# ShuoYangRobotics/Cerberus

Measured on NVIDIA H100. Metric: sliding-window solves/sec (10-frame x 150-feature windows), higher is better.
Workload: dtype f64

## Files before the change

cerberus_b200/csrc/solve_kernel.cuh:

```cuda
#pragma once
#include "eval_kernels.cuh"

namespace cerb {

#if defined(CERB_PHASE_TIMING) && !defined(CERB_CUSIM)
__device__ unsigned long long g_phase_cycles[48];
#define PH_DECL() long long ph_t = clock64()
#define PH_MARK_T(id, t) do { if ((threadIdx.x & 31) == 0) { const long long ph_n = clock64(); if (threadIdx.x == (t)) atomicAdd(&g_phase_cycles[id], (unsigned long long)(ph_n - ph_t)); ph_t = ph_n; } __syncwarp(); } while (0)
#define PH_MARK(id) PH_MARK_T(id, 0)
#define PH_ARG , long long &ph_t
#define PH_FWD , ph_t
#else
#define PH_DECL()
#define PH_MARK_T(id, t)
#define PH_MARK(id)
#define PH_ARG
#define PH_FWD
#endif

enum { CERB_WINDOW = 10, NX = 79, NYB = 13, NFR = 11, NY = 143, NR = 222, NRP = 224, HXX_SZ = 79 * 79, HXY_SZ = 79 * 143, X_TD = 78, SOLVE_THREADS = 256, FT = 64, TILE_LD = 33, NOBS_PLANES = 9 };
enum { HBLK = NYB * NYB, AD_SZ = NFR * HBLK, BO_SZ = (NFR - 1) * HBLK };
#ifndef CERB_SOLVE_MIN_BLOCKS
#define CERB_SOLVE_MIN_BLOCKS 1
#endif
// ... 629 lines not shown
                    _Pragma("unroll")
                    for (int t = 0; t < 15; t++) {
                        const int o = plx[hq + t] + i * (ply[hq + t] & 4095);
                        const double nv = cur[t] + acc[(hq + t) >> 1][(hq + t) & 1];
                        smem_base[o] = nv;
                        smem_base[o + (ply[hq + t] >> 12) - 256] = nv;
                    }
                }
                PH_MARK(35);
            } else if (i + 1 < CERB_WINDOW && rnd < 3) load_S(i + 1);
            CERB_BAR_SYNC(2, 32 * IMU_WARPS);
            PH_MARK(36);
        }
        PH_MARK(30);
    } else {
        const int *meta = P.prior_meta + (size_t)w * PRIOR_META_STRIDE;
        if (meta[0]) {
            const int t5 = tid - 32 * IMU_WARPS, n = meta[1], nb = meta[2];
            const double *J = P.prior_J + (size_t)w * PRIOR_LD * PRIOR_LD, *r0 = P.prior_r + (size_t)w * PRIOR_LD, *x0 = P.prior_x0 + (size_t)w * 16 * 9;
            if (t5 < nb) {
                const int kind = meta[4 + 3 * t5], index = meta[5 + 3 * t5], col = meta[6 + 3 * t5];
                prior_block_dx(kind, x + prior_block_state_offset(kind, index), x0 + 9 * t5, s.pdx + col);
            }
            CERB_BAR_SYNC(3, PRIOR_THREADS);
            const int kc = (n + 1) / 2;
            for (int e = t5; e < 2 * n; e += PRIOR_THREADS) {
                const int p = e / n, i = e % n;
                const int k1 = (p + 1) * kc < n ? (p + 1) * kc : n;
                double t = 0.0;
                for (int k = p * kc; k < k1; k++) t += J[(size_t)k * n + i] * s.pdx[k];
                ppart[p * PRIOR_LD + i] = t;
            }
            CERB_BAR_SYNC(3, PRIOR_THREADS);
            for (int i = t5; i < n; i += PRIOR_THREADS) {
                const double t = (r0[i] + ppart[i]) + ppart[PRIOR_LD + i];
                s.pr[i] = t; cost += 0.5 * t * t;
            }
            CERB_BAR_SYNC(3, PRIOR_THREADS);
            for (int c = wid - IMU_WARPS; c < n; c += PRIOR_THREADS / 32) {
                double t = 0.0;
                for (int k = lane; k < n; k += 32) t += J[(size_t)c * n + k] * s.pr[k];
                for (int o = 16; o > 0; o >>= 1) t += __shfl_sync(0xffffffffu, t, (lane + o) & 31);
                const int d = s.ti[TI_PRIOR_MAP + c];
                if (lane == 0) gp[d >= 0 ? d : NX + (-d - 1)] += t;
            }
        }
        PH_MARK_T(31, 96);
    }
    __syncthreads();
    PH_MARK(26);
    for (int k = tid; k < NR; k += SOLVE_THREADS) s.g[k] += gp[k];
    __syncthreads();
    PH_MARK(27);
    return cost;
}

CERB_D void apply_plus(const Smem &s, const double *delta, const double *lam, const double *dlam, double *lamc, int nF, bool ex_open, bool td_open, int tid) {
    if (tid < 11) pose_plus(s.xs + ST_POSE + 7 * tid, delta + 6 * tid, s.xc + ST_POSE + 7 * tid);
    else if (tid < 13) {
        const int e = tid - 11;
        if (ex_open) pose_plus(s.xs + ST_EX + 7 * e, delta + 66 + 6 * e, s.xc + ST_EX + 7 * e);
        else for (int k = 0; k < 7; k++) s.xc[ST_EX + 7 * e + k] = s.xs[ST_EX + 7 * e + k];
    }
    for (int k = tid; k < 99; k += SOLVE_THREADS) { const int f = k / 9, c = k % 9; s.xc[ST_SB + k] = s.xs[ST_SB + k] + delta[NX + NYB * f + c]; }
    for (int k = tid; k < 44; k += SOLVE_THREADS) { const int f = k / 4, c = k % 4; s.xc[ST_LB + k] = s.xs[ST_LB + k] + delta[NX + NYB * f + 9 + c]; }
    if (tid == 0) s.xc[ST_TD] = td_open ? s.xs[ST_TD] + delta[X_TD] : s.xs[ST_TD];
    for (int f = tid; f < nF; f += SOLVE_THREADS) lamc[f] = lam[f] + dlam[f];
    __syncthreads();
}

CERB_D double ambient_sq(const double *a, const double *b, const double *la, const double *lb, int nF, bool ex_open, bool lb_open, bool td_open, int tid) {
    double t = 0.0;
    for (int k = tid; k < ST_SIZE; k += SOLVE_THREADS) {
        if (k >= ST_LB && k < ST_EX && !lb_open) continue;
        if (k >= ST_EX && k < ST_TD && !ex_open) continue;
        if (k == ST_TD && !td_open) continue;
        const double v = b ? a[k] - b[k] : a[k];
        t += v * v;
    }
    for (int f = tid; f < nF; f += SOLVE_THREADS) { const double v = lb ? la[f] - lb[f] : la[f]; t += v * v; }
    return t;
}

template <int W> struct TTPlan;
#define CERB_TT_PLAN(W, NR_, NB_, ...) template <> struct TTPlan<W> { static constexpr int nr = NR_, nb = NB_; static CERB_HD int tab(int i) { constexpr int t[] = {__VA_ARGS__}; return t[i]; } };
CERB_TT_PLAN(0, 4, 7, 0, 1, 2, 3, 0, 0, 0,   0, 0, 1, 0, 1, 0, 1,   0, 1, 1, 2, 2, 3, 3)
CERB_TT_PLAN(1, 4, 7, 2, 3, 4, 5, 0, 0, 0,   0, 0, 1, 0, 1, 0, 1,   0, 1, 1, 2, 2, 3, 3)
CERB_TT_PLAN(2, 4, 7, 4, 5, 6, 7, 0, 0, 0,   0, 0, 1, 0, 1, 0, 1,   0, 1, 1, 2, 2, 3, 3)
CERB_TT_PLAN(3, 4, 7, 6, 7, 8, 9, 0, 0, 0,   0, 0, 1, 0, 1, 0, 1,   0, 1, 1, 2, 2, 3, 3)
CERB_TT_PLAN(4, 6, 7, 8, 9, 0, 1, 4, 5, 0,   0, 0, 1, 2, 3, 2, 3,   0, 1, 1, 4, 4, 5, 5)
CERB_TT_PLAN(5, 6, 7, 0, 1, 6, 7, 8, 9, 0,   0, 0, 0, 0, 1, 1, 1,   2, 3, 4, 5, 2, 3, 4)
CERB_TT_PLAN(6, 7, 7, 1, 9, 2, 6, 7, 8, 3,   0, 2, 2, 2, 2, 6, 6,   1, 3, 4, 5, 1, 3, 4)
CERB_TT_PLAN(7, 5, 6, 3, 4, 5, 8, 9, 0, 0,   0, 0, 1, 1, 2, 2, 0,   3, 4, 3, 4, 3, 4, 0)
template <int W> CERB_D void ttt_warp(Smem &s, int lane) {
    typedef TTPlan<W> PL;
    const double *pr[7];
    _Pragma("unroll")
    for (int u = 0; u < 7; u++) {
        const int r = 8 * PL::tab(u < PL::nr ? u : 0) + (lane >> 2);
        pr[u] = (r < NX ? s.Hxy + r * NY : s.yv + NX) + (lane & 3);
    }
    double acc[7][2], fv[7];
    _Pragma("unroll")
    for (int k = 0; k < 7; k++) { acc[k][0] = 0.0; acc[k][1] = 0.0; }
    _Pragma("unroll")
    for (int u = 0; u < 7; u++) fv[u] = (u < PL::nr) ? pr[u][0] : 0.0;
    for (int q0 = 0; q0 < NY; q0 += 4) {
        const int qn = q0 + 4;
        const bool take = qn < NY && qn + (lane & 3) < NY;
        double fn[7];
        _Pragma("unroll")
        for (int u = 0; u < 7; u++) fn[u] = (u < PL::nr && take) ? pr[u][qn] : 0.0;
        _Pragma("unroll")
        for (int k = 0; k < 7; k++) if (k < PL::nb) CERB_DMMA(acc[k][0], acc[k][1], fv[PL::tab(7 + k)], fv[PL::tab(14 + k)], acc[k][0], acc[k][1]);
        _Pragma("unroll")
        for (int u = 0; u < 7; u++) fv[u] = fn[u];
    }
    _Pragma("unroll")
    for (int k = 0; k < 7; k++) {
        if (k >= PL::nb) continue;
        const int ba = PL::tab(PL::tab(7 + k)), bb = PL::tab(PL::tab(14 + k));
        const int a = 8 * ba + (lane >> 2);
        for (int e = 0; e < 2; e++) {
            const int b = 8 * bb + 2 * (lane & 3) + e;
            if (a > b || a >= NX || b > NX) continue;
            if (b == NX) s.yv[a] -= acc[k][e];
            else s.Hxx[b * NX + a] -= acc[k][e];
        }
    }
}

template <int W> struct SCPlan;
#define CERB_SC_PLAN(W, NR_, NB_, ...) template <> struct SCPlan<W> { static constexpr int nr = NR_, nb = NB_; static CERB_HD int tab(int i) { constexpr int t[] = {__VA_ARGS__}; return t[i]; } };
CERB_SC_PLAN(0, 8, 8, 0, 1, 2, 3, 4, 5, 6, 7, 0,   0, 0, 0, 0, 0, 0, 0, 0,   0, 1, 2, 3, 4, 5, 6, 7)
CERB_SC_PLAN(1, 9, 8, 0, 8, 9, 1, 2, 3, 4, 5, 6,   0, 0, 3, 3, 3, 3, 3, 3,   1, 2, 3, 4, 5, 6, 7, 8)
CERB_SC_PLAN(2, 9, 8, 1, 7, 8, 9, 2, 3, 4, 5, 6,   0, 0, 0, 4, 4, 4, 4, 4,   1, 2, 3, 4, 5, 6, 7, 8)
CERB_SC_PLAN(3, 8, 8, 2, 7, 8, 9, 3, 4, 5, 6, 0,   0, 0, 0, 4, 4, 4, 4, 4,   1, 2, 3, 4, 5, 6, 7, 1)
CERB_SC_PLAN(4, 7, 8, 3, 8, 9, 4, 5, 6, 7, 0, 0,   0, 0, 3, 3, 3, 3, 3, 3,   1, 2, 3, 4, 5, 6, 1, 2)
CERB_SC_PLAN(5, 5, 8, 5, 6, 7, 8, 9, 0, 0, 0, 0,   0, 0, 0, 0, 0, 1, 1, 1,   0, 1, 2, 3, 4, 1, 2, 3)
CERB_SC_PLAN(6, 4, 7, 6, 7, 8, 9, 0, 0, 0, 0, 0,   0, 1, 1, 1, 2, 2, 3, 0,   3, 1, 2, 3, 2, 3, 3, 0)
enum { SC_LDW = 36 };
template <int W> CERB_D void schur_tile(const double *tw, double (&acc)[8][2], int lane) {
    typedef SCPlan<W> PL;
    const double *pr[9];
    _Pragma("unroll")
    for (int u = 0; u < 9; u++) pr[u] = tw + (8 * PL::tab(u < PL::nr ? u : 0) + (lane >> 2)) * SC_LDW + (lane & 3);
    double fv[9];
    _Pragma("unroll")
    for (int u = 0; u < 9; u++) fv[u] = (u < PL::nr) ? pr[u][0] : 0.0;
    _Pragma("unroll")
    for (int ks = 0; ks < 8; ks++) {
        double fn[9];
        _Pragma("unroll")
        for (int u = 0; u < 9; u++) fn[u] = (u < PL::nr && ks < 7) ? pr[u][4 * (ks + 1)] : 0.0;
        _Pragma("unroll")
        for (int k = 0; k < 8; k++) if (k < PL::nb) CERB_DMMA(acc[k][0], acc[k][1], fv[PL::tab(9 + k)], fv[PL::tab(17 + k)], acc[k][0], acc[k][1]);
        _Pragma("unroll")
        for (int u = 0; u < 9; u++) fv[u] = fn[u];
    }
}
template <int W> CERB_D void schur_scatter(Smem &s, const double (&acc)[8][2], int lane) {
    typedef SCPlan<W> PL;
    _Pragma("unroll")
    for (int k = 0; k < 8; k++) {
        if (k >= PL::nb) continue;
        const int a = 8 * PL::tab(PL::tab(9 + k)) + (lane >> 2);
// ... 160 lines not shown
        const double D = sqrt(fmin(fmax(d, 1e-6), 1e32));
        s.D[k] = D; s.gh[k] = s.g[k] / D; s.stp[k] = s.gh[k] / D;
    }
    for (int f = tid; f < nF; f += SOLVE_THREADS) { const double D = sqrt(fmin(fmax(c.ws.hh[f], 1e-6), 1e32)); Dl[f] = D; ghl[f] = c.ws.gl[f] / D; stl[f] = ghl[f] / D; }
    __syncthreads();
    double part[2] = {0.0, 0.0};
    for (int k = tid; k < AD_SZ; k += SOLVE_THREADS) { const int f = k / HBLK, a = (k % HBLK) / NYB, b = k % NYB; part[0] += s.stp[NX + NYB * f + a] * s.Ad[k] * s.stp[NX + NYB * f + b]; }
    for (int k = tid; k < BO_SZ; k += SOLVE_THREADS) { const int f = k / HBLK, a = (k % HBLK) / NYB, b = k % NYB; part[0] += 2.0 * s.stp[NX + NYB * f + a] * s.Bo[k] * s.stp[NX + NYB * (f + 1) + b]; }
    for (int f = tid; f < nF; f += SOLVE_THREADS) part[1] += ghl[f] * ghl[f];
    for (int k = tid; k < NR; k += SOLVE_THREADS) part[1] += s.gh[k] * s.gh[k];
    double tot[2];
    block_sum<2>(part, s.red, tot, tid);
    if (tid == 0) { sca[S_GNORM2] = tot[1]; sca[S_VHV] = tot[0]; sca[S_OK] = 1; }
    PH_MARK(4);
}
CERB_D void chain_cholesky(Smem &s, int *chain_done, int lane PH_ARG) {
    const bool act = lane < NYB;
    const int r = act ? lane : 0;
    double m[NYB];
    _Pragma("unroll")
    for (int c = 0; c < NYB; c++) m[c] = 0.0;
    _Pragma("unroll 1")
    for (int f = 0; f < NFR; f++) {
        double *A = s.Ad + f * HBLK;
        double a[NYB], invd[NYB], myinv = 1.0;
        _Pragma("unroll")
        for (int c = 0; c < NYB; c++) a[c] = A[r * NYB + c];
        if (f > 0) {
            const double *Mp = s.Bo + (f - 1) * HBLK;
            _Pragma("unroll")
            for (int c = 0; c < NYB; c++) { double t = 0.0; _Pragma("unroll") for (int q = 0; q < NYB; q++) t += m[q] * Mp[c * NYB + q]; a[c] -= t; }
        }
        _Pragma("unroll")
        for (int j = 0; j < NYB; j++) {
            double d = __shfl_sync(0xffffffffu, a[j], j);
            if (!(d > 0.0)) { if (lane == 0) s.sca[S_OK] = 0; d = 1.0; }
            const double inv = rsqrt(d);
            invd[j] = inv;
            if (lane == j) myinv = inv;
            const double l = (lane == j) ? d * inv : a[j] * inv;
            a[j] = l;
            double *colb = s.chain_col + 16 * (j & 1);
            if (act) colb[lane] = l;
            __syncwarp();
            _Pragma("unroll")
            for (int k = j + 1; k < NYB; k++) a[k] -= l * colb[k];
        }
        if (act) { _Pragma("unroll") for (int c = 0; c < NYB; c++) if (c <= r) A[r * NYB + c] = a[c]; s.idg[NYB * f + r] = myinv; }
        __syncwarp();
        if (f < NFR - 1) {
            double *B = s.Bo + f * HBLK;
            double t[NYB];
            _Pragma("unroll")
            for (int c = 0; c < NYB; c++) t[c] = B[c * NYB + r];
            _Pragma("unroll")
            for (int c = 0; c < NYB; c++) {
                m[c] = t[c] * invd[c];
                _Pragma("unroll")
                for (int c2 = c + 1; c2 < NYB; c2++) t[c2] -= m[c] * A[c2 * NYB + c];
            }
            __syncwarp();
            if (act) { _Pragma("unroll") for (int c = 0; c < NYB; c++) B[r * NYB + c] = m[c]; }
            __syncwarp();
        }
        __threadfence_block(); __syncwarp();
        if (lane == 0) CERB_ST_RELEASE_S32(chain_done, f + 1);
    }
    PH_MARK(6);
}
CERB_D void schur_tile_w(int wq, const double *tw, double (&acc)[8][2], int lane) {
    switch (wq) { case 0: schur_tile<0>(tw, acc, lane); break; case 1: schur_tile<1>(tw, acc, lane); break; case 2: schur_tile<2>(tw, acc, lane); break;
                  case 3: schur_tile<3>(tw, acc, lane); break; case 4: schur_tile<4>(tw, acc, lane); break; case 5: schur_tile<5>(tw, acc, lane); break;
                  default: schur_tile<6>(tw, acc, lane); break; }
}
CERB_D void schur_scatter_w(int wq, Smem &s, const double (&acc)[8][2], int lane) {
    switch (wq) { case 0: schur_scatter<0>(s, acc, lane); break; case 1: schur_scatter<1>(s, acc, lane); break; case 2: schur_scatter<2>(s, acc, lane); break;
                  case 3: schur_scatter<3>(s, acc, lane); break; case 4: schur_scatter<4>(s, acc, lane); break; case 5: schur_scatter<5>(s, acc, lane); break;
                  default: schur_scatter<6>(s, acc, lane); break; }
}
CERB_D void ttt_warp_w(int wq, Smem &s, int lane) {
    switch (wq) { case 0: ttt_warp<0>(s, lane); break; case 1: ttt_warp<1>(s, lane); break; case 2: ttt_warp<2>(s, lane); break; case 3: ttt_warp<3>(s, lane); break;
                  case 4: ttt_warp<4>(s, lane); break; case 5: ttt_warp<5>(s, lane); break; case 6: ttt_warp<6>(s, lane); break; default: ttt_warp<7>(s, lane); break; }
}
CERB_D void lambda_schur(Smem &s, const Win &c, double mu, int tid PH_ARG) {
    const int F = c.ws.F, nF = c.nF;
    const double *W = c.ws.W, *hh = c.ws.hh, *gl = c.ws.gl, *Dl = c.ws.Dl, *stl = c.ws.stl;
    const int t2 = tid - 32, n2 = SOLVE_THREADS - 32;
    const int wq = (tid >> 5) - 1, lane = tid & 31;
    const int LDW = SC_LDW;
    double *tw = s.Ju;
    double *sinv = nF <= 1024 ? s.wj : c.ws.sinv;
    {
        const double *v = s.stp;
        double pv = 0.0;
        for (int k = t2; k < NX * NX; k += n2) pv += v[k / NX] * s.Hxx[k] * v[k % NX];
        for (int k = t2; k < NX * NY; k += n2) pv += 2.0 * v[k / NY] * s.Hxy[k] * v[NX + k % NY];
        for (int f = t2; f < nF; f += n2) {
            double wv = 0.0;
            for (int a = 0; a < NX; a++) wv += W[(size_t)a * F + f] * v[a];
            pv += 2.0 * stl[f] * wv + hh[f] * stl[f] * stl[f];
        }
        for (int o = 16; o > 0; o >>= 1) pv += __shfl_sync(0xffffffffu, pv, (lane + o) & 31);
        if (lane == 0) s.lin[wq] = pv;
        CERB_BAR_SYNC(1, n2);
        for (int k = t2; k < NX; k += n2) s.Hxx[k * NX + k] += mu * s.D[k] * s.D[k];
    }
    PH_MARK_T(19, 32);
    for (int f = t2; f < nF; f += n2) sinv[f] = rsqrt(hh[f] + mu * Dl[f] * Dl[f]);
    double acc[8][2];
    _Pragma("unroll")
    for (int k = 0; k < 8; k++) { acc[k][0] = 0.0; acc[k][1] = 0.0; }
    CERB_BAR_SYNC(1, n2);
    double buf[12];
    auto fetch = [&](int f0) {
        const int nf = (nF - f0) < 32 ? (nF - f0) : 32;
        _Pragma("unroll")
        for (int u = 0; u < 12; u++) {
            const int e = t2 + u * n2, a = e >> 5, f = e & 31;
            buf[u] = (e < 80 * 32 && f < nf) ? (a < NX ? W[(size_t)a * F + f0 + f] : (a == NX ? gl[f0 + f] : 0.0)) : 0.0;
        }
    };
    fetch(0);
    PH_MARK_T(37, 32);
    for (int f0 = 0; f0 < nF; f0 += 32) {
        const int nf = (nF - f0) < 32 ? (nF - f0) : 32;
        _Pragma("unroll")
        for (int u = 0; u < 12; u++) {
            const int e = t2 + u * n2, a = e >> 5, f = e & 31;
            if (e < 80 * 32) tw[a * LDW + f] = (f < nf) ? buf[u] * sinv[f0 + f] : 0.0;
        }
        CERB_BAR_SYNC(1, n2);
        PH_MARK_T(38, 32);
        if (f0 + 32 < nF) fetch(f0 + 32);
        schur_tile_w(wq, tw, acc, lane);
        CERB_BAR_SYNC(1, n2);
        PH_MARK_T(39, 32);
    }
    schur_scatter_w(wq, s, acc, lane);
    PH_MARK_T(7, 32);
}
CERB_D void forward_subst(Smem &s, const int *chain_done, int t2) {
    if (t2 <= NX) {
        double *row = (t2 < NX) ? s.Hxy + t2 * NY : s.yv + NX;
        double tp[NYB];
        _Pragma("unroll")
        for (int k = 0; k < NYB; k++) tp[k] = 0.0;
        _Pragma("unroll 1")
        for (int f = 0; f < NFR; f++) {
            while (CERB_LD_ACQUIRE_S32(chain_done) <= f) { CERB_SPIN_PAUSE(); }
            __threadfence_block();
            const double *L = s.Ad + f * HBLK, *idg = s.idg + NYB * f;
            double *t = row + NYB * f;
            double tc[NYB];
            _Pragma("unroll")
            for (int r = 0; r < NYB; r++) tc[r] = t[r];
            if (f > 0) {
                const double *M = s.Bo + (f - 1) * HBLK;
                _Pragma("unroll")
                for (int r = 0; r < NYB; r++) { double acc = 0.0; _Pragma("unroll") for (int q = 0; q < NYB; q++) acc += M[r * NYB + q] * tp[q]; tc[r] -= acc; }
            }
            _Pragma("unroll")
            for (int c = 0; c < NYB; c++) {
                tc[c] *= idg[c];
                _Pragma("unroll")
                for (int r = c + 1; r < NYB; r++) tc[r] -= L[r * NYB + c] * tc[c];
            }
            _Pragma("unroll")
            for (int r = 0; r < NYB; r++) { t[r] = tc[r]; tp[r] = tc[r]; }
        }
    }
}
CERB_D void panel_cholesky(Smem &s, int tid) {
    const int wq = tid >> 5, lane = tid & 31;
    auto factor_diag = [&](int c0, int nb, double *Lkk) {
        const bool act = lane < nb;
        const int r = act ? lane : 0;
        double a[8];
        _Pragma("unroll")
        for (int c = 0; c < 8; c++) a[c] = (c < nb && c <= r) ? s.Hxx[(c0 + r) * NX + c0 + c] : 0.0;
        double myinv = 1.0;
        _Pragma("unroll")
        for (int j = 0; j < 8; j++) {
            double d = __shfl_sync(0xffffffffu, a[j], j);
            if (j < nb && !(d > 0.0)) { if (lane == 0) s.sca[S_OK] = 0; }
            if (!(d > 0.0)) d = 1.0;
            const double inv = rsqrt(d);
            if (lane == j) myinv = inv;
            const double l = (lane == j) ? d * inv : a[j] * inv;
            a[j] = l;
            _Pragma("unroll")
            for (int k = j + 1; k < 8; k++) { const double lk = __shfl_sync(0xffffffffu, l, k); a[k] -= l * lk; }
        }
        if (act) {
            _Pragma("unroll")
            for (int c = 0; c < 8; c++) if (c <= r) { s.Hxx[(c0 + r) * NX + c0 + c] = a[c]; Lkk[r * 8 + c] = a[c]; }
            Lkk[64 + r] = myinv; s.idx[c0 + r] = myinv;
        }
    };
    auto trailing_block = [&](int c0, int b0, int b) {
        int bi = 0, idx = b;
        while (idx > bi) { idx -= bi + 1; bi++; }
        const int ri = 8 * (b0 + bi) + (lane >> 2), rj = 8 * (b0 + idx) + (lane >> 2);
        double a0 = 0.0, a1 = 0.0;
        for (int ks = 0; ks < 2; ks++) {
            const int cc = c0 + 4 * ks + (lane & 3);
            const double av = (ri < NX) ? s.Hxx[ri * NX + cc] : (ri == NX ? s.yv[cc] : 0.0);
            const double bv = (rj < NX) ? s.Hxx[rj * NX + cc] : 0.0;
            CERB_DMMA(a0, a1, av, bv, a0, a1);
        }
        const int cj = 8 * (b0 + idx) + 2 * (lane & 3);
        if (ri < NX) {
            if (cj <= ri && cj < NX) s.Hxx[ri * NX + cj] -= a0;
            if (cj + 1 <= ri && cj + 1 < NX) s.Hxx[ri * NX + cj + 1] -= a1;
        } else if (ri == NX) {
            if (cj < NX) s.yv[cj] -= a0;
            if (cj + 1 < NX) s.yv[cj + 1] -= a1;
        }
    };
    if (wq == 0) factor_diag(0, 8, s.red);
    __syncthreads();
    int pk = 0;
    for (int c0 = 0; c0 < NX; c0 += 8, pk ^= 1) {
        const int nb = (NX - c0) < 8 ? (NX - c0) : 8, c1 = c0 + nb;
        const double *Lkk = s.red + 80 * pk;
        if (tid <= NX - c1) {
            const int i = c1 + tid;
            double *row = (i < NX) ? s.Hxx + i * NX + c0 : s.yv + c0;
            double t[8];
            _Pragma("unroll")
            for (int c = 0; c < 8; c++) t[c] = (c < nb) ? row[c] : 0.0;
            _Pragma("unroll")
            for (int c = 0; c < 8; c++) {
                if (c < nb) {
                    t[c] *= Lkk[64 + c];
                    _Pragma("unroll")
                    for (int c2 = c + 1; c2 < 8; c2++) if (c2 < nb) t[c2] -= t[c] * Lkk[c2 * 8 + c];
                }
            }
            _Pragma("unroll")
            for (int c = 0; c < 8; c++) if (c < nb) row[c] = t[c];
        }
        __syncthreads();
        if (c1 >= NX) break;
        {
            const int b0 = c1 >> 3, nbt = 10 - b0;
            const int nblk = nbt * (nbt + 1) / 2;
            if (wq == 0) {
                trailing_block(c0, b0, 0);
                __syncwarp();
                factor_diag(c1, (NX - c1) < 8 ? (NX - c1) : 8, s.red + 80 * (pk ^ 1));
            } else {
                for (int b = wq; b < nblk; b += 7) trailing_block(c0, b0, b);
            }
        }
        __syncthreads();
    }
}
CERB_D void back_substitution(const SolveParams &P, Smem &s, const Win &c, PriorCopy &pc, double mu, int &gn_attempts, int tid PH_ARG) {
    if (tid < 32) {
        double y0 = s.yv[tid], y1 = s.yv[32 + tid], y2 = (64 + tid < NX) ? s.yv[64 + tid] : 0.0;
        _Pragma("unroll 1")
        for (int k = NX - 1; k >= 0; k--) {
            const double *Lk = s.Hxx + k * NX;
            const double ik = s.idx[k];
            const double l0 = (tid < k) ? Lk[tid] : 0.0, l1 = (32 + tid < k) ? Lk[32 + tid] : 0.0, l2 = (64 + tid < k) ? Lk[64 + tid] : 0.0;
            const double src = (k >= 64) ? y2 : (k >= 32 ? y1 : y0);
            const double yk = __shfl_sync(0xffffffffu, src, k & 31) * ik;
            y0 = (tid == k) ? yk : y0 - l0 * yk;
            y1 = (32 + tid == k) ? yk : y1 - l1 * yk;
            y2 = (64 + tid == k) ? yk : y2 - l2 * yk;
        }
        s.yv[tid] = y0; s.yv[32 + tid] = y1; if (64 + tid < NX) s.yv[64 + tid] = y2;
    }
    __syncthreads();
    if (c.has_prior) {
        if (c.bulk_ok) { if (tid == 0) CERB_BULK_G2S(s.Hxx, c.ws.pimg, PIMG_HXY * 8, &s.mbar[0]); }
        else copy_g2s_async(s.Hxx, c.ws.pimg, HXX_SZ, tid);
        pc.hxx_prefetched = true;
    }
    PH_MARK(11);
    for (int q = tid; q < NY; q += SOLVE_THREADS) { double t = 0.0; for (int a = 0; a < NX; a++) t += s.Hxy[a * NY + q] * s.yv[a]; s.yv[NX + q] -= t; }
    __syncthreads();
    if (tid < 32) {
        const int r = tid < NYB ? tid : 0;
        double yn[NYB];
        _Pragma("unroll")
        for (int k = 0; k < NYB; k++) yn[k] = 0.0;
        _Pragma("unroll 1")
        for (int f = NFR - 1; f >= 0; f--) {
            const double *L = s.Ad + f * HBLK;
            double u = s.yv[NX + NYB * f + r];
            if (f < NFR - 1) {
                const double *M = s.Bo + f * HBLK;
                double t = 0.0;
                _Pragma("unroll")
                for (int k = 0; k < NYB; k++) t += M[k * NYB + r] * yn[k];
                u -= t;
            }
            double lc[NYB], ig[NYB];
            _Pragma("unroll")
            for (int k = 0; k < NYB; k++) { lc[k] = (tid < k) ? L[k * NYB + r] : 0.0; ig[k] = s.idg[NYB * f + k]; }
            _Pragma("unroll")
            for (int k = NYB - 1; k >= 0; k--) {
                const double yk = __shfl_sync(0xffffffffu, u, k) * ig[k];
                yn[k] = yk;
                u = (tid == k) ? yk : u - lc[k] * yk;
            }
            if (tid < NYB) s.yv[NX + NYB * f + tid] = u;
        }
    }
    __syncthreads();
    PH_MARK(12);
    double bad = 0.0;
    for (int f = tid; f < c.nF; f += SOLVE_THREADS) {
        double t = c.ws.gl[f];
        for (int a = 0; a < NX; a++) t -= c.ws.W[(size_t)a * c.ws.F + f] * s.yv[a];
        const double y = t / (c.ws.hh[f] + mu * c.ws.Dl[f] * c.ws.Dl[f]);
        c.ws.gnl[f] = y;
        if (!(fabs(y) < 1e300)) bad = 1.0;
    }
    for (int k = tid; k < NR; k += SOLVE_THREADS) if (!(fabs(s.yv[k]) < 1e300)) bad = 1.0;
    if (bad != 0.0) s.sca[S_OK] = 0;
    if (gn_attempts < P.test_fail_factorizations) s.sca[S_OK] = 0;
    gn_attempts++;
    __syncthreads();
    PH_MARK(13);
}
CERB_D void gauss_newton_step(const SolveParams &P, Smem &s, const Win &c, PriorCopy &pc, int &gn_attempts, int tid PH_ARG) {
    const int nF = c.nF;
    const double mu = s.sca[S_MU];
    for (int k = tid; k < NR; k += SOLVE_THREADS) {
        s.yv[k] = s.g[k];
        if (k >= NX) s.Ad[((k - NX) / NYB) * HBLK + ((k - NX) % NYB) * (NYB + 1)] += mu * s.D[k] * s.D[k];
    }
    int *chain_done = s.ti + TI_CHAIN_DONE;
    if (tid == 0) *chain_done = 0;
    __syncthreads();
    if (tid < 32) chain_cholesky(s, chain_done, tid PH_FWD);
    else { lambda_schur(s, c, mu, tid PH_FWD); forward_subst(s, chain_done, tid - 32); }
    __syncthreads();
    if (tid == 0) {
        double vhv = s.sca[S_VHV];
        for (int k = 0; k < 7; k++) vhv += s.lin[k];
        s.sca[S_ALPHA] = s.sca[S_GNORM2] / vhv;
    }
    PH_MARK(5);
    __syncthreads();
    PH_MARK(8);
    ttt_warp_w(tid >> 5, s, tid & 31);
    __syncthreads();
    PH_MARK(9);
    panel_cholesky(s, tid);
    PH_MARK(10);
    back_substitution(P, s, c, pc, mu, gn_attempts, tid PH_FWD);
    if (s.sca[S_OK] != 0.0) {
        double part3[2] = {0.0, 0.0};
        for (int k = tid; k < NR; k += SOLVE_THREADS) { const double v = -s.D[k] * s.yv[k]; s.gn[k] = v; part3[0] += v * v; part3[1] += s.gh[k] * v; }
        for (int f = tid; f < nF; f += SOLVE_THREADS) { const double v = -c.ws.Dl[f] * c.ws.gnl[f]; c.ws.gnl[f] = v; part3[0] += v * v; part3[1] += c.ws.ghl[f] * v; }
        double tot3[2];
        block_sum<2>(part3, s.red, tot3, tid);
        if (tid == 0) { s.sca[S_GNNORM2] = tot3[0]; s.sca[S_GDOTGN] = tot3[1]; }
        __syncthreads();
    }
}
CERB_D void dogleg_step(double *sca, int tid) {
    if (tid == 0) {
        const double radius = sca[S_RADIUS], alpha = sca[S_ALPHA];
        const double gradient_norm = sqrt(sca[S_GNORM2]), gauss_newton_norm = sqrt(sca[S_GNNORM2]);
        double p, q, nrm;
        if (gauss_newton_norm <= radius) { p = 0.0; q = 1.0; nrm = gauss_newton_norm; }
        else if (gradient_norm * alpha >= radius) { p = -(radius / gradient_norm); q = 0.0; nrm = radius; }
        else {
            const double b_dot_a = -alpha * sca[S_GDOTGN];
            const double a_squared_norm = (alpha * gradient_norm) * (alpha * gradient_norm);
            const double b_minus_a_squared_norm = a_squared_norm - 2 * b_dot_a + gauss_newton_norm * gauss_newton_norm;
            const double c = b_dot_a - a_squared_norm;
            const double d = sqrt(c * c + b_minus_a_squared_norm * (radius * radius - a_squared_norm));
            const double beta = (c <= 0) ? (d - c) / b_minus_a_squared_norm : (radius * radius - a_squared_norm) / (d + c);
            p = -alpha * (1.0 - beta); q = beta;
            nrm = sqrt(p * p * sca[S_GNORM2] + 2 * p * q * sca[S_GDOTGN] + q * q * sca[S_GNNORM2]);
        }
        sca[S_P] = p; sca[S_Q] = q; sca[S_DLNORM] = nrm;
        const double mu = sca[S_MU], g2 = sca[S_GNORM2], gg = sca[S_GDOTGN], n2 = sca[S_GNNORM2];
        const double sTg = p * g2 + q * gg;
        const double sHs = p * p * (g2 / alpha) - 2.0 * p * q * (g2 + mu * gg) + q * q * (-gg - mu * n2);
        sca[S_MODEL] = -(sTg + 0.5 * sHs);
    }
    __syncthreads();
}
CERB_D bool handle_invalid_step(double *sca, int tid) {
    if (tid == 0) {
        sca[S_INVALID] += 1;
        if (sca[S_INVALID] >= 5) { sca[S_DONE] = 1; sca[S_TERM] = 2; }
        sca[S_MU] *= 10.0; sca[S_REUSE] = 0;
    }
    __syncthreads();
    return sca[S_DONE] != 0.0;
}
CERB_D void evaluate_candidate(const SolveParams &P, Smem &s, const Win &c, PriorCopy &pc, bool speculate, int tid PH_ARG) {
    const int nF = c.nF;
    double *sca = s.sca, *stl = c.ws.stl, *lamc = c.ws.lamc;
    {
        const double p = sca[S_P], q = sca[S_Q];
        for (int k = tid; k < NR; k += SOLVE_THREADS) s.stp[k] = (p * s.gh[k] + q * s.gn[k]) / s.D[k] * s.sc[k];
        for (int f = tid; f < nF; f += SOLVE_THREADS) stl[f] = (p * c.ws.ghl[f] + q * c.ws.gnl[f]) / c.ws.Dl[f] * c.ws.sl[f];
    }
    __syncthreads();
    PH_MARK(14);
    apply_plus(s, s.stp, c.lam, stl, lamc, nF, c.ex_open, c.td_open, tid);
    double part[2];
    PH_MARK(15);
    if (speculate) { linearize(P, s, c, pc, s.xc, lamc, false, tid PH_FWD); part[0] = 0.0; }
    else {
        load_geometry(s.xc, s, tid);
        part[0] = vision_cost(P, c.w, s.xc, lamc, tid);
        PH_MARK(16);
        part[0] += inertial_cost(P, c.w, s.xc, tid);
    }
    PH_MARK(17);
    part[1] = ambient_sq(s.xs, s.xc, c.lam, lamc, nF, c.ex_open, c.lb_open, c.td_open, tid);
    double tot[2];
    block_sum<2>(part, s.red, tot, tid);
    if (tid == 0) {
        double cc = speculate ? sca[S_LCOST] : tot[0];
        if (!(cc == cc) || fabs(cc) > 1e300) cc = 1.7976931348623157e308;
        sca[S_CCOST] = cc; sca[S_STEPNORM] = sqrt(tot[1]);
    }
    __syncthreads();
}
CERB_D bool accept_or_reject(const SolveParams &P, double *sca, int tid) {
    if (tid == 0) {
        const double x_cost = sca[S_XCOST], cand = sca[S_CCOST];
        if (sca[S_STEPNORM] <= P.ptol * (sca[S_XNORM] + P.ptol)) { sca[S_DONE] = 1; sca[S_TERM] = 0; }
        else if (fabs(x_cost - cand) <= P.ftol * x_cost) { sca[S_DONE] = 1; sca[S_TERM] = 0; }
        else {
            const double rel = (x_cost - cand) / sca[S_MODEL];
            if (rel > P.min_rel_dec) {
// ... 240 lines not shown
```

cerberus_b200/estimator.py:

```python
import ctypes as C
import numpy as np
from . import abi

WINDOW_SIZE = abi.WINDOW_SIZE
FOCAL_LENGTH = 460.0
MIN_PARALLAX = 10.0 / FOCAL_LENGTH
INIT_DEPTH = 5.0
MARGIN_OLD, MARGIN_SECOND_NEW = 0, 1


def quat_to_R(q):
    x, y, z, w = q
    tx, ty, tz = 2 * x, 2 * y, 2 * z
    twx, twy, twz, txx, txy, txz, tyy, tyz, tzz = tx * w, ty * w, tz * w, tx * x, ty * x, tz * x, ty * y, tz * y, tz * z
    return np.array([[1 - (tyy + tzz), txy - twz, txz + twy], [txy + twz, 1 - (txx + tzz), tyz - twx], [txz - twy, tyz + twx, 1 - (txx + tyy)]])


def R_to_quat(m):
    t = m[0, 0] + m[1, 1] + m[2, 2]
    q = np.zeros(4)
    if t > 0:
        t = np.sqrt(t + 1.0); q[3] = 0.5 * t; t = 0.5 / t
        q[0], q[1], q[2] = (m[2, 1] - m[1, 2]) * t, (m[0, 2] - m[2, 0]) * t, (m[1, 0] - m[0, 1]) * t
    else:
# ... 400 lines not shown
        T["marginalize"] += time.perf_counter() - t0
        for w, e in enumerate(self.est):
            e.prior = take_prior(self.batch_next, w) if self.batch_next.descs[w].prior.valid else (e.prior if flags[w] == MARGIN_SECOND_NEW else None)
        t0 = time.perf_counter()
        err = self.ops.outlier_errors(self.batch)
        T["outliers"] += time.perf_counter() - t0
        t0 = time.perf_counter()
        for w, e in enumerate(self.est):
            bad = {fid for k, fid in enumerate(ids[w]) if err[w, k] * FOCAL_LENGTH > 3}
            if bad: e.f_manager.removeOutlier(bad)
        ids2 = [fill_window(self.batch_all, w, e, min_used=1, with_prior=False) for w, e in enumerate(self.est)]
        for w, e in enumerate(self.est):
            lam = self.batch_all.para_Feature[w]
            for k, it in enumerate(e.f_manager.feature): lam[k] = 1.0 / it.estimated_depth
        T["host"] += time.perf_counter() - t0
        t0 = time.perf_counter()
        _, sdepth, _ = self.ops.shift_depth(self.batch_all)
        T["shift"] += time.perf_counter() - t0
        t0 = time.perf_counter()
        for w, e in enumerate(self.est):
            e.slide_window({fid: float(sdepth[w, k]) for k, fid in enumerate(ids2[w])})
            e.f_manager.removeFailures()
            W = WINDOW_SIZE
            e.path.append((header, e.Ps[W].copy(), e.Rs[W].copy(), e.Vs[W].copy(), e.Rho[W].copy()))
        T["host"] += time.perf_counter() - t0
        return rep

    def run(self, seq, n_steps=None):
        self.seed(seq)
        last = seq.n_frames if n_steps is None else min(seq.n_frames, WINDOW_SIZE + n_steps)
        for k in range(WINDOW_SIZE, last):
            if k == WINDOW_SIZE:
                firsts = [seq.first[w, k - 1] for w in range(self.n)]; smp = [seq.samples[w, k - 1][:0] for w in range(self.n)]
            else:
                firsts = [seq.first[w, k - 1] for w in range(self.n)]; smp = [seq.samples[w, k - 1] for w in range(self.n)]
            self.step([seq.images[k][w] for w in range(self.n)], firsts, smp, float(k))
        return self

    def poses(self):
        P = np.array([[p[1] for p in e.path] for e in self.est]); R = np.array([[p[2] for p in e.path] for e in self.est])
        return P, R


class DeviceOps:

    def __init__(self, backend, cfg):
        self.be, self.cfg = backend, cfg

    def preintegrate(self, pcfg, jobs, n): return self.be.preintegrate(pcfg, jobs, n)
    def preintegrate_imu(self, pcfg, jobs, n): return self.be.preintegrate_imu(pcfg, jobs, n)
    def solve(self, batch): return self.be.solve_batch(batch)
    def double2vector(self, before, after): return self.be.double2vector(before, after)

    def triangulate(self, batch):
        self.be.upload(batch)
        return self.be.triangulate(batch.n, INIT_DEPTH)[:, :batch.max_features]

    def outlier_errors(self, batch):
        self.be.upload(batch)
        return self.be.outlier_errors(batch.n, FOCAL_LENGTH)[0][:, :batch.max_features]

    def shift_depth(self, batch):
        self.be.upload(batch)
        a, b, c = self.be.shift_depth(batch.n, INIT_DEPTH)
        F = batch.max_features
        return a[:, :F], b[:, :F], c[:, :F]

    def marginalize(self, src, dst, flags):
        self.be.marginalize(self.cfg, src, dst, margin_old=(np.asarray(flags) == MARGIN_OLD))


class NativeReplay:

    def __init__(self, backend, pcfg, n, max_features=160, estimate_extrinsic=1, estimate_td=0, resident=False):
        self.be, self.n = backend, n
        self.r = C.c_void_p()
        backend._check(backend.lib.cerb_replay_create(backend.h, C.byref(pcfg), n, max_features, estimate_extrinsic, estimate_td, C.byref(self.r)))
        if resident:
            backend._check(backend.lib.cerb_replay_set_resident(self.r, 1))
        self.reports = []

    def close(self):
        if self.r:
            self.be.lib.cerb_replay_destroy(self.r); self.r = C.c_void_p()

    def __del__(self):
        try: self.close()
        except Exception: pass

    @staticmethod
    def _image(img, keep):
        ids = np.ascontiguousarray(img["ids"], dtype=np.int64); p0 = np.ascontiguousarray(img["pts0"], dtype=np.float64)
        h1 = np.ascontiguousarray(img["has1"], dtype=np.uint8); p1 = np.ascontiguousarray(img["pts1"], dtype=np.float64)
        keep.extend([ids, p0, h1, p1])
        im = abi.Image(); im.n = len(ids)
        im.ids = ids.ctypes.data_as(C.POINTER(C.c_int64)); im.pts0 = p0.ctypes.data_as(abi.c_dp); im.has1 = h1.ctypes.data_as(C.POINTER(C.c_uint8)); im.pts1 = p1.ctypes.data_as(abi.c_dp)
        return im

    def seed(self, seq):
        for w in range(self.n):
            self.seed_robot(w, seq, w)

    def seed_robot(self, robot, seq, w, k0=0):
        L, _p = self.be.lib, lambda a: np.ascontiguousarray(a, dtype=np.float64).ctypes.data_as(abi.c_dp)
        tic, ric = np.ascontiguousarray(seq.tic_g[w]), np.ascontiguousarray(seq.ric_g[w])
        self.be._check(L.cerb_replay_set_extrinsics(self.r, robot, _p(tic), _p(ric)))
        for k in range(WINDOW_SIZE + 1):
            keep, K = [], k0 + k
            first = np.ascontiguousarray(seq.first[w, K if k == 0 else K - 1: (K + 1 if k == 0 else K)])
            smp = np.ascontiguousarray(seq.samples[w][K - 1]) if k > 0 else first[:0]
            im = self._image(seq.images[K][w], keep) if k < WINDOW_SIZE else None
            P, R, V = np.ascontiguousarray(seq.p_g[w, K]), np.ascontiguousarray(seq.R_g[w, K]), np.ascontiguousarray(seq.v_g[w, K])
            self.be._check(L.cerb_replay_seed_frame(self.r, robot, k, _p(P), _p(R), _p(V), first.ctypes.data, smp.ctypes.data if len(smp) else None, len(smp),
                                                    C.byref(im) if im is not None else None, float(K)))

    def configure(self, robot, use_leg, pcfg, estimate_extrinsic=1, estimate_td=0):
        self.be._check(self.be.lib.cerb_replay_configure_robot(self.r, robot, 1 if use_leg else 0, C.byref(pcfg), estimate_extrinsic, estimate_td))

    def reset(self, robot):
        self.be._check(self.be.lib.cerb_replay_reset_robot(self.r, robot))

    def step(self, images, firsts, samples, header, robots=None, headers=None):
        keep = []
        m = self.n if robots is None else len(robots)
        ims = (abi.Image * m)(*[self._image(images[i], keep) for i in range(m)])
        fr = np.ascontiguousarray(np.stack([np.asarray(firsts[i]).reshape(()) for i in range(m)]))
        smp = [np.ascontiguousarray(samples[i]) for i in range(m)]
        ptrs = (C.c_void_p * m)(*[s.ctypes.data if len(s) else None for s in smp])
        ns = (C.c_int32 * m)(*[len(s) for s in smp])
        rep = (abi.SolveReport * m)()
        if robots is None and headers is None:
            self.be._check(self.be.lib.cerb_replay_step(self.r, ims, fr.ctypes.data, ptrs, ns, float(header), rep))
        else:
            rob = np.ascontiguousarray(np.arange(self.n) if robots is None else robots, dtype=np.int32)
            hdr = np.ascontiguousarray(np.full(m, float(header)) if headers is None else headers, dtype=np.float64)
            self.be._check(self.be.lib.cerb_replay_step_robots(self.r, m, rob.ctypes.data_as(C.POINTER(C.c_int32)), ims, fr.ctypes.data, ptrs, ns,
                                                               hdr.ctypes.data_as(abi.c_dp), rep))
        self.reports.append(np.frombuffer(rep, dtype=abi.report_dtype, count=m).copy())

    def run(self, seq, n_steps=None):
        self.seed(seq)
        last = seq.n_frames if n_steps is None else min(seq.n_frames, WINDOW_SIZE + n_steps)
        for k in range(WINDOW_SIZE, last):
            firsts = [seq.first[w, k - 1] for w in range(self.n)]
            smp = [seq.samples[w][k - 1][:0] if k == WINDOW_SIZE else seq.samples[w][k - 1] for w in range(self.n)]
            self.step([seq.images[k][w] for w in range(self.n)], firsts, smp, float(k))
        return self

    def path(self, w):
        n = C.c_int32()
        self.be._check(self.be.lib.cerb_replay_path(self.r, w, C.byref(n), None, 0))
        out = np.zeros((n.value, 20))
        self.be._check(self.be.lib.cerb_replay_path(self.r, w, C.byref(n), out.ctypes.data_as(abi.c_dp), n.value))
        return out

    def poses(self):
        rows = np.stack([self.path(w) for w in range(self.n)])
        return rows[:, :, 1:4], rows[:, :, 4:13].reshape(self.n, -1, 3, 3)

    def feature_ids(self, w):
        n = C.c_int32(); ids = np.zeros(4096, dtype=np.int32)
        self.be._check(self.be.lib.cerb_replay_feature_ids(self.r, w, C.byref(n), ids.ctypes.data_as(C.POINTER(C.c_int32)), ids.size))
        return ids[:n.value].tolist()

    def flag_history(self, w):
        n = C.c_int32(); out = np.zeros(4096, dtype=np.int32)
        self.be._check(self.be.lib.cerb_replay_flags(self.r, w, C.byref(n), out.ctypes.data_as(C.POINTER(C.c_int32)), out.size))
# ... 34 lines not shown
```

Baseline: 29170.

## Split GN solve into noinline stages and batch strided W column loads

Moves the elimination, reduce/factor and back-substitution phases into separate noinline device functions. Each one re-carves shared memory from the dynamic base, which is meant to cut register pressure and live state across the big solve function. It also adds a helper that loads W columns in batches of 16 before the dot products, so more global loads are in flight at once. Function-call overhead and re-deriving pointers cost a little, and the estimator gains a null-handle guard on destroy.

```diff
diff --git a/cerberus_b200/csrc/solve_kernel.cuh b/cerberus_b200/csrc/solve_kernel.cuh
--- a/cerberus_b200/csrc/solve_kernel.cuh
+++ b/cerberus_b200/csrc/solve_kernel.cuh
@@ -735,6 +735,21 @@
     return t;
 }
 
+template <bool SUB>
+CERB_D double w_column_dot(const double *wf, int F, const double *v, double t) {
+    constexpr int BATCH = 16;
+    for (int a0 = 0; a0 < NX; a0 += BATCH) {
+        double wr[BATCH];
+        _Pragma("unroll")
+        for (int u = 0; u < BATCH; u++) wr[u] = (a0 + u < NX) ? wf[(size_t)(a0 + u) * F] : 0.0;
+        _Pragma("unroll")
+        for (int u = 0; u < BATCH; u++) {
+            if (a0 + u < NX) { if (SUB) t -= wr[u] * v[a0 + u]; else t += wr[u] * v[a0 + u]; }
+        }
+    }
+    return t;
+}
+
 template <int W> struct TTPlan;
 #define CERB_TT_PLAN(W, NR_, NB_, ...) template <> struct TTPlan<W> { static constexpr int nr = NR_, nb = NB_; static CERB_HD int tab(int i) { constexpr int t[] = {__VA_ARGS__}; return t[i]; } };
 CERB_TT_PLAN(0, 4, 7, 0, 1, 2, 3, 0, 0, 0,   0, 0, 1, 0, 1, 0, 1,   0, 1, 1, 2, 2, 3, 3)
@@ -1061,22 +1076,21 @@
     switch (wq) { case 0: ttt_warp<0>(s, lane); break; case 1: ttt_warp<1>(s, lane); break; case 2: ttt_warp<2>(s, lane); break; case 3: ttt_warp<3>(s, lane); break;
                   case 4: ttt_warp<4>(s, lane); break; case 5: ttt_warp<5>(s, lane); break; case 6: ttt_warp<6>(s, lane); break; default: ttt_warp<7>(s, lane); break; }
 }
-CERB_D void lambda_schur(Smem &s, const Win &c, double mu, int tid PH_ARG) {
-    const int F = c.ws.F, nF = c.nF;
-    const double *W = c.ws.W, *hh = c.ws.hh, *gl = c.ws.gl, *Dl = c.ws.Dl, *stl = c.ws.stl;
+CERB_D void lambda_schur(Smem &s, const CtaWs &ws, int nF, double mu, int tid PH_ARG) {
+    const int F = ws.F;
+    const double *W = ws.W, *hh = ws.hh, *gl = ws.gl, *Dl = ws.Dl, *stl = ws.stl;
     const int t2 = tid - 32, n2 = SOLVE_THREADS - 32;
     const int wq = (tid >> 5) - 1, lane = tid & 31;
     const int LDW = SC_LDW;
     double *tw = s.Ju;
-    double *sinv = nF <= 1024 ? s.wj : c.ws.sinv;
+    double *sinv = nF <= 1024 ? s.wj : ws.sinv;
     {
         const double *v = s.stp;
         double pv = 0.0;
         for (int k = t2; k < NX * NX; k += n2) pv += v[k / NX] * s.Hxx[k] * v[k % NX];
         for (int k = t2; k < NX * NY; k += n2) pv += 2.0 * v[k / NY] * s.Hxy[k] * v[NX + k % NY];
         for (int f = t2; f < nF; f += n2) {
-            double wv = 0.0;
-            for (int a = 0; a < NX; a++) wv += W[(size_t)a * F + f] * v[a];
+            const double wv = w_column_dot<false>(W + f, F, v, 0.0);
             pv += 2.0 * stl[f] * wv + hh[f] * stl[f] * stl[f];
         }
         for (int o = 16; o > 0; o >>= 1) pv += __shfl_sync(0xffffffffu, pv, (lane + o) & 31);
@@ -1235,7 +1249,26 @@
         __syncthreads();
     }
 }
-CERB_D void back_substitution(const SolveParams &P, Smem &s, const Win &c, PriorCopy &pc, double mu, int &gn_attempts, int tid PH_ARG) {
+CERB_NOINLINE void gn_eliminate(const SolveParams &P, int w, double mu, int tid PH_ARG) {
+    CERB_DYN_SMEM(double, smem_base);
+    Smem s; smem_carve(smem_base, s);
+    int *chain_done = s.ti + TI_CHAIN_DONE;
+    if (tid < 32) chain_cholesky(s, chain_done, tid PH_FWD);
+    else { lambda_schur(s, ws_carve(P), P.n_features[w], mu, tid PH_FWD); forward_subst(s, chain_done, tid - 32); }
+}
+CERB_NOINLINE void gn_reduce_factor(int tid PH_ARG) {
+    CERB_DYN_SMEM(double, smem_base);
+    Smem s; smem_carve(smem_base, s);
+    ttt_warp_w(tid >> 5, s, tid & 31);
+    __syncthreads();
+    PH_MARK(9);
+    panel_cholesky(s, tid);
+    PH_MARK(10);
+}
+CERB_NOINLINE void back_substitution(const SolveParams &P, int w, bool has_prior, bool bulk_ok, double mu, bool fail, int tid PH_ARG) {
+    CERB_DYN_SMEM(double, smem_base);
+    Smem s; smem_carve(smem_base, s);
+    const CtaWs ws = ws_carve(P);
     if (tid < 32) {
         double y0 = s.yv[tid], y1 = s.yv[32 + tid], y2 = (64 + tid < NX) ? s.yv[64 + tid] : 0.0;
         _Pragma("unroll 1")
@@ -1252,10 +1285,9 @@
         s.yv[tid] = y0; s.yv[32 + tid] = y1; if (64 + tid < NX) s.yv[64 + tid] = y2;
     }
     __syncthreads();
-    if (c.has_prior) {
-        if (c.bulk_ok) { if (tid == 0) CERB_BULK_G2S(s.Hxx, c.ws.pimg, PIMG_HXY * 8, &s.mbar[0]); }
-        else copy_g2s_async(s.Hxx, c.ws.pimg, HXX_SZ, tid);
-        pc.hxx_prefetched = true;
+    if (has_prior) {
+        if (bulk_ok) { if (tid == 0) CERB_BULK_G2S(s.Hxx, ws.pimg, PIMG_HXY * 8, &s.mbar[0]); }
+        else copy_g2s_async(s.Hxx, ws.pimg, HXX_SZ, tid);
     }
     PH_MARK(11);
     for (int q = tid; q < NY; q += SOLVE_THREADS) { double t = 0.0; for (int a = 0; a < NX; a++) t += s.Hxy[a * NY + q] * s.yv[a]; s.yv[NX + q] -= t; }
@@ -1291,17 +1323,16 @@
     __syncthreads();
     PH_MARK(12);
     double bad = 0.0;
-    for (int f = tid; f < c.nF; f += SOLVE_THREADS) {
-        double t = c.ws.gl[f];
-        for (int a = 0; a < NX; a++) t -= c.ws.W[(size_t)a * c.ws.F + f] * s.yv[a];
-        const double y = t / (c.ws.hh[f] + mu * c.ws.Dl[f] * c.ws.Dl[f]);
-        c.ws.gnl[f] = y;
+    const int nF = P.n_features[w];
+    for (int f = tid; f < nF; f += SOLVE_THREADS) {
+        const double t = w_column_dot<true>(ws.W + f, ws.F, s.yv, ws.gl[f]);
+        const double y = t / (ws.hh[f] + mu * ws.Dl[f] * ws.Dl[f]);
+        ws.gnl[f] = y;
         if (!(fabs(y) < 1e300)) bad = 1.0;
     }
     for (int k = tid; k < NR; k += SOLVE_THREADS) if (!(fabs(s.yv[k]) < 1e300)) bad = 1.0;
     if (bad != 0.0) s.sca[S_OK] = 0;
-    if (gn_attempts < P.test_fail_factorizations) s.sca[S_OK] = 0;
-    gn_attempts++;
+    if (fail) s.sca[S_OK] = 0;
     __syncthreads();
     PH_MARK(13);
 }
@@ -1312,11 +1343,9 @@
         s.yv[k] = s.g[k];
         if (k >= NX) s.Ad[((k - NX) / NYB) * HBLK + ((k - NX) % NYB) * (NYB + 1)] += mu * s.D[k] * s.D[k];
     }
-    int *chain_done = s.ti + TI_CHAIN_DONE;
-    if (tid == 0) *chain_done = 0;
-    __syncthreads();
-    if (tid < 32) chain_cholesky(s, chain_done, tid PH_FWD);
-    else { lambda_schur(s, c, mu, tid PH_FWD); forward_subst(s, chain_done, tid - 32); }
+    if (tid == 0) s.ti[TI_CHAIN_DONE] = 0;
+    __syncthreads();
+    gn_eliminate(P, c.w, mu, tid PH_FWD);
     __syncthreads();
     if (tid == 0) {
         double vhv = s.sca[S_VHV];
@@ -1326,12 +1355,10 @@
     PH_MARK(5);
     __syncthreads();
     PH_MARK(8);
-    ttt_warp_w(tid >> 5, s, tid & 31);
-    __syncthreads();
-    PH_MARK(9);
-    panel_cholesky(s, tid);
-    PH_MARK(10);
-    back_substitution(P, s, c, pc, mu, gn_attempts, tid PH_FWD);
+    gn_reduce_factor(tid PH_FWD);
+    back_substitution(P, c.w, c.has_prior, c.bulk_ok, mu, gn_attempts < P.test_fail_factorizations, tid PH_FWD);
+    if (c.has_prior) pc.hxx_prefetched = true;
+    gn_attempts++;
     if (s.sca[S_OK] != 0.0) {
         double part3[2] = {0.0, 0.0};
         for (int k = tid; k < NR; k += SOLVE_THREADS) { const double v = -s.D[k] * s.yv[k]; s.gn[k] = v; part3[0] += v * v; part3[1] += s.gh[k] * v; }
diff --git a/cerberus_b200/estimator.py b/cerberus_b200/estimator.py
--- a/cerberus_b200/estimator.py
+++ b/cerberus_b200/estimator.py
@@ -506,7 +506,9 @@
 
     def close(self):
         if self.r:
-            self.be.lib.cerb_replay_destroy(self.r); self.r = C.c_void_p()
+            if self.be.h:
+                self.be.lib.cerb_replay_destroy(self.r)
+            self.r = C.c_void_p()
 
     def __del__(self):
         try: self.close()
```

Result: faster. 33510 (median of 6 runs) (+14.9%).
